# bchess/k8s-1m

Measured on AMD Instinct MI355X. Metric: pods scheduled/sec at 1M nodes (1/2/4/8 GPU) + % of HBM roofline, higher is better.
Workload: dtype int64+f64

## Files before the change

k8s-1m_amd/csrc/ksched_eval.hpp:

```cpp
#pragma once

#include <hip/hip_runtime.h>

#include "ksched_dev.hpp"

namespace ks {

struct NodeRegs {
  double free_cpu, free_mem;
  double rcpu, rmem;
  double lf100_cpu, lf100_mem;
  double acpu_d, amem_d;
  double inv_cpu, inv_mem;
  double bamul;
  uint32_t slot;
  uint32_t bits;
  uint32_t lashift;
};

__device__ __forceinline__ NodeRegs make_regs_inv(int64_t acpu, int64_t amem, int64_t rc, int64_t rm, int64_t zc,
                                                  int64_t zm, int32_t apods, int32_t np, uint32_t slot,
                                                  double inv_cpu, double inv_mem) {
  NodeRegs r;
  r.slot = slot;
// ... 183 lines not shown
  const uint32_t rb = __builtin_amdgcn_readfirstlane(f.rcp_both), rc = __builtin_amdgcn_readfirstlane(f.rcp_cpu),
                 rm = __builtin_amdgcn_readfirstlane(f.rcp_mem);
  const bool hc = r.inv_cpu != 0.0, hm = r.inv_mem != 0.0;
  const uint32_t rcp = hc ? (hm ? rb : rc) : rm;
  return (int32_t)__umulhi(n << 1, rcp);
}

__device__ __forceinline__ uint32_t *fit_table_lds() {
  __shared__ uint32_t s_fit_table[FIT_TABLE_WORDS];
  return s_fit_table;
}
__device__ __forceinline__ void fit_table_stage(const uint32_t *table) {
  if (threadIdx.x < FIT_TABLE_WORDS) fit_table_lds()[threadIdx.x] = table[threadIdx.x];
}
__device__ __forceinline__ int32_t score_fit_rtcr(double nz100_cpu, double nz100_mem, const NodeRegs &r,
                                                  const FitParams &f, const uint8_t *T) {
  const uint32_t uc = min(fit_resource(true, r.lf100_cpu, nz100_cpu, r.acpu_d, r.inv_cpu), 100u);
  const uint32_t um = min(fit_resource(true, r.lf100_mem, nz100_mem, r.amem_d, r.inv_mem), 100u);
  const uint32_t tc = r.inv_cpu != 0.0 ? (uint32_t)T[uc] : 0u, tm = r.inv_mem != 0.0 ? (uint32_t)T[um] : 0u;
  const uint32_t rb = __builtin_amdgcn_readfirstlane(f.rcp_both), rc = __builtin_amdgcn_readfirstlane(f.rcp_cpu),
                 rm = __builtin_amdgcn_readfirstlane(f.rcp_mem);
  return (int32_t)fit_rtcr_node_score(tc, tm, f.wc, f.wm, rc, rm, rb);
}

template <int GF>
__device__ __forceinline__ int32_t score_fit_nz(double nz100_cpu, double nz100_mem, const NodeRegs &r,
                                                const FitParams &f) {
  static_assert(GF == 1 || GF == 2, "the default strategy scores a PodDev (score_la)");
  if constexpr (GF == 2) return score_fit_rtcr(nz100_cpu, nz100_mem, r, f, (const uint8_t *)fit_table_lds());
  else return score_fit_general(nz100_cpu, nz100_mem, r, f);
}
template <int GF>
__device__ __forceinline__ int32_t score_fit(const PodDev &p, const NodeRegs &r, const FitParams &f) {
  if constexpr (GF == 0) return score_la(p, r);
  else return score_fit_nz<GF>(p.nz100_cpu, p.nz100_mem, r, f);
}

template <int GF>
__device__ __forceinline__ void fit_x_resource(FitXSum &x, uint32_t w, int64_t cap, int64_t req, const FitParams &f,
                                               const uint8_t *T) {
  static_assert(GF == 1 || GF == 2, "the default strategy lists no extended resource");
  if constexpr (GF == 2) {
    const uint32_t u = min(fit_x_score(true, cap, req), 100u);
    fit_x_add_rtcr(x, w, cap ? (uint32_t)T[u] : 0u);
  } else {
    fit_x_add(x, w, fit_x_score(f.most != 0, cap, req), cap != 0);
  }
}
template <int GF>
__device__ __forceinline__ int32_t score_fit_x(const PodDev &p, const NodeRegs &r, const FitParams &f, FitXSum x,
                                               const uint32_t *xrcp, const uint8_t *T) {
  if constexpr (GF == 2) {
    const uint32_t uc = min(fit_resource(true, r.lf100_cpu, p.nz100_cpu, r.acpu_d, r.inv_cpu), 100u);
    const uint32_t um = min(fit_resource(true, r.lf100_mem, p.nz100_mem, r.amem_d, r.inv_mem), 100u);
    fit_x_add_rtcr(x, f.wc, r.inv_cpu != 0.0 ? (uint32_t)T[uc] : 0u);
    fit_x_add_rtcr(x, f.wm, r.inv_mem != 0.0 ? (uint32_t)T[um] : 0u);
    return (int32_t)fit_x_round_div(x.n, x.d);
  } else {
    const uint32_t sc = fit_resource(f.most, r.lf100_cpu, p.nz100_cpu, r.acpu_d, r.inv_cpu);
    const uint32_t sm = fit_resource(f.most, r.lf100_mem, p.nz100_mem, r.amem_d, r.inv_mem);
    const uint32_t n = x.n + wmad(f.wc, sc, wmul(f.wm, sm));
    const bool hc = r.inv_cpu != 0.0, hm = r.inv_mem != 0.0;
    const uint32_t rcp = hc ? (hm ? xrcp[3] : xrcp[1]) : (hm ? xrcp[2] : xrcp[0]);
    return (int32_t)fit_x_div(n, rcp);
  }
}

__device__ __forceinline__ double div_rn(double a, double b, double y) {
  const double q0 = a * y;
  const double r = __builtin_fma(-b, q0, a);
  return __builtin_fma(r, y, q0);
}

__device__ __forceinline__ int32_t score_ba_sum(double sc, double sm, const NodeRegs &r) {
  const double f0 = fmin(div_rn(sc, r.acpu_d, r.inv_cpu), 1.0);
  const double f1 = fmin(div_rn(sm, r.amem_d, r.inv_mem), 1.0);
  const double om = __builtin_fma(-fabs(f0 - f1), r.bamul, 1.0);
  return (int32_t)(om * 100.0);
}

__device__ __forceinline__ double ba_fraction(double s, double alloc, double inv) {
  return fmin(div_rn(s, alloc, inv), 1.0);
}
__device__ __forceinline__ int32_t score_ba_fractions(double f0, double f1, const NodeRegs &r) {
  const double om = __builtin_fma(-fabs(f0 - f1), r.bamul, 1.0);
  return (int32_t)(om * 100.0);
}
__device__ __forceinline__ int32_t score_la_cpu(int32_t la_cpu, double nz100_mem, const NodeRegs &r) {
  return (la_cpu + least_requested(r.lf100_mem, nz100_mem, r.inv_mem)) >> r.lashift;
}

__device__ __forceinline__ int32_t score_ba(const PodDev &p, const NodeRegs &r) {
  return score_ba_sum(r.rcpu + p.req_cpu_d, r.rmem + p.req_mem_d, r);
}

__device__ __forceinline__ int64_t taint_raw(const PodDev &p, const NodeExt &e) {
  return (int64_t)__popcll(e.prefer & ~p.tol_prefer);
}

__device__ __forceinline__ int64_t normalize(int64_t raw, int64_t mx, bool reverse) {
  if (mx == 0) return reverse ? 100 : 0;
  const int64_t s = (int64_t)((uint32_t)(100 * raw) / (uint32_t)mx);
  return reverse ? 100 - s : s;
}

template <bool EXT, int GF>
__device__ __forceinline__ int32_t total_score(const PodDev &p, const uint64_t *clauses, const NodeRegs &r,
                                               const NodeExt &e, const Weights &w, const FitParams &fs,
                                               int64_t tt_max, int64_t na_max) {
  int32_t t = (int32_t)wmul((uint32_t)w.fit, (uint32_t)score_fit<GF>(p, r, fs)) +
              (int32_t)wmul((uint32_t)w.ba, (uint32_t)score_ba(p, r));
  int32_t tt = 100;
  if (EXT && (p.flags & PF_TT)) tt = (int32_t)normalize(taint_raw(p, e), tt_max, true);
  t += w.tt * tt;
  if (p.flags & PF_HAS_PREF) {
    int32_t na = 0;
    if (EXT && (p.flags & PF_NA)) na = (int32_t)normalize(preferred_raw(p, clauses, e, r.slot), na_max, false);
    t += (int32_t)wmul((uint32_t)w.na, (uint32_t)na);
  }
  return t;
}

__device__ __forceinline__ uint64_t pack_key(int64_t total, uint32_t slot) {
  return ((uint64_t)(total + 1) << 32) | (uint64_t)(0xFFFFFFFFu - slot);
}

__device__ __forceinline__ void ext_from_words(const uint64_t *w, NodeExt &e) {
  e.hard = w[0];
  e.prefer = w[1];
#pragma unroll
  for (int q = 0; q < LW; ++q) e.lab[q] = w[2 + q];
#pragma unroll
  for (int q = 0; q < NNUM; ++q) e.num[q] = (int64_t)w[2 + LW + q];
}

template <bool EXT>
__device__ __forceinline__ void status_delta(const PodDev &p, const uint64_t *clauses, int st0, int st1,
                                            const NodeExt &e, uint32_t slot, int64_t tt_max, int64_t na_max,
                                            int32_t *d) {
  d[0] += (st0 == ST_FEASIBLE) - (st1 == ST_FEASIBLE);
#pragma unroll
  for (int q = 0; q < NFILT; ++q) d[1 + q] += (st1 == q) - (st0 == q);
  if (EXT && (p.flags & PF_TT)) {
    const int at = taint_raw(p, e) == tt_max;
    d[6] += (st0 == ST_FEASIBLE) * at - (st1 == ST_FEASIBLE) * at;
  }
  if (EXT && (p.flags & PF_NA)) {
    const int at = preferred_raw(p, clauses, e, slot) == na_max;
    d[7] += (st0 == ST_FEASIBLE) * at - (st1 == ST_FEASIBLE) * at;
  }
}

}
```

k8s-1m_amd/csrc/ksched_kernels.hip:

```cpp
#include <hip/hip_runtime.h>

#include <utility>

#include "ksched_dev.hpp"
#include "ksched_eval.hpp"
#include "ksched_kernels.hpp"
#include "ksched_instr.hpp"
#include "ksched_util.hpp"

namespace ks {




typedef unsigned u32x4 __attribute__((ext_vector_type(4)));
typedef const __attribute__((address_space(4))) u32x4 *const_words;
template <bool SCALAR = false>
__device__ __forceinline__ PodDev load_pod(const PodDev *pods, uint32_t i) {
  if constexpr (SCALAR) {
    const const_words src = (const_words)(pods + i);
    u32x4 w[sizeof(PodDev) / 16];
#pragma unroll
    for (int k = 0; k < (int)(sizeof(PodDev) / 16); ++k) w[k] = src[k];
    PodDev p;
    __builtin_memcpy(&p, w, sizeof p);
    return p;
  } else {
    return pods[i];
  }
}


template <typename T>
__device__ __forceinline__ void pin_vgpr(T &x) {
  asm volatile("" : "+v"(x));
}

template <int NPL, int LWU>
__device__ __forceinline__ const uint64_t *term_pass_n(const uint64_t *t, const NodeExt (&e)[NPL],
                                                       const NodeRegs (&nr)[NPL], uint32_t (&ok)[NPL]) {
  const uint64_t w0 = t[0];
  const uint32_t ng = uniform_u32((uint32_t)w0 & 0xFF), nn = uniform_u32(((uint32_t)w0 >> 8) & 0xFF),
                 nm = uniform_u32(((uint32_t)w0 >> 16) & 0xFF);
  uint64_t must[LWU], mf[LWU];
#pragma unroll
  for (int k = 0; k < LWU; ++k) {
    must[k] = t[1 + k];
    mf[k] = t[1 + LW + k];
  }
  static_for<NPL>([&](auto J) {
    constexpr int j = J;
    uint64_t diff = 0;
#pragma unroll
    for (int k = 0; k < LWU; ++k) diff |= (e[j].lab[k] & mf[k]) ^ must[k];
    ok[j] = diff == 0 ? 1u : 0u;
  });
  const uint64_t *g = t + TERM_HDR_WORDS;
  for (uint32_t i = 0; i < ng; ++i, g += LW) {
    uint64_t gm[LWU];
#pragma unroll
    for (int k = 0; k < LWU; ++k) gm[k] = g[k];
    static_for<NPL>([&](auto J) {
      constexpr int j = J;
      uint64_t any = 0;
#pragma unroll
      for (int k = 0; k < LWU; ++k) any |= e[j].lab[k] & gm[k];
      ok[j] &= any != 0 ? 1u : 0u;
    });
  }
  for (uint32_t i = 0; i < nn; ++i, g += 2) {
    const bool col1 = g[0] & 0xFF, gt = ((g[0] >> 8) & 0xFF) == TO_GT;
    const int64_t x = (int64_t)g[1];
    static_for<NPL>([&](auto J) {
      constexpr int j = J;
      const int64_t v = col1 ? e[j].num[1] : e[j].num[0];
      ok[j] &= (gt ? v > x : v < x) ? 1u : 0u;
    });
  }
  for (uint32_t i = 0; i < nm; ++i, g += 2) {
    const bool in = g[0] == TO_NAME_IN;
    const int64_t x = (int64_t)g[1];
    static_for<NPL>([&](auto J) {
      constexpr int j = J;
      ok[j] &= (((int64_t)nr[j].slot == x) == in) ? 1u : 0u;
    });
  }
  return g;
}

template <int NPL, int LWU>
__device__ __forceinline__ void required_match_n(const PodDev &p, const uint64_t *prog, const NodeExt (&e)[NPL],
                                                 const NodeRegs (&nr)[NPL], bool (&out)[NPL]) {
  uint32_t any[NPL];
  static_for<NPL>([&](auto J) { any[J] = 0u; });
  const uint64_t *t = prog + p.req_off;
  for (uint32_t k = 0; k < p.req_len; ++k) {
    uint32_t ok[NPL];
    t = term_pass_n<NPL, LWU>(t, e, nr, ok);
    static_for<NPL>([&](auto J) { any[J] |= ok[J]; });
  }
  static_for<NPL>([&](auto J) { out[J] = any[J] != 0u; });
}

template <int NPL, int LWU>
__device__ __forceinline__ void preferred_raw_n(const PodDev &p, const uint64_t *prog, const NodeExt (&e)[NPL],
                                                const NodeRegs (&nr)[NPL], uint32_t (&raw)[NPL]) {
  static_for<NPL>([&](auto J) { raw[J] = 0u; });
  const uint64_t *t = prog + p.pref_off;
  for (uint32_t k = 0; k < p.pref_len; ++k) {
    const uint32_t w = uniform_u32((uint32_t)(t[0] >> 32));
    uint32_t ok[NPL];
    t = term_pass_n<NPL, LWU>(t, e, nr, ok);
    static_for<NPL>([&](auto J) { raw[J] += ok[J] * w; });
  }
}

constexpr double NORM_EPS = 0x1p-40;
__device__ __forceinline__ uint32_t normalize_inv(uint32_t raw, double inv) {
  return (uint32_t)__builtin_fma((double)(100u * raw), inv, NORM_EPS);
}


constexpr uint32_t KEY32_POS_BITS = 9, KEY32_POS_MASK = (1u << KEY32_POS_BITS) - 1;
static_assert(((uint64_t)KS_MAX_PLUGIN_WEIGHT << KEY32_POS_BITS) < (1ull << 24), "pre-shifted weight: 24-bit operand");
static_assert((((uint64_t)4 * 100 * KS_MAX_PLUGIN_WEIGHT + 1) << KEY32_POS_BITS) + KEY32_POS_MASK < (1ull << 31),
              "the sweep's 32-bit key");

template <int NPL, bool EXT, int LWU = LW, int GF = 0>
__global__ __launch_bounds__(SWEEP_THREADS) __attribute__((amdgpu_waves_per_eu(EXT && NPL == 2 && !GF ? 5 : 1)))
void sweep_kernel(RoundArgs a) {
  static_assert(NPL * WAVE <= (1 << KEY32_POS_BITS), "wave-local key position field");
  constexpr int NW = SWEEP_THREADS / WAVE;
  __shared__ uint64_t s_keys[MAX_PG][NW][3];
  constexpr int NCNT = NFILT + 5;
  __shared__ uint32_t s_cnt[MAX_PG][NW][NCNT];
  __shared__ uint64_t s_stage[EXT ? 1 : NW][EXT ? 1 : WL_T][EXT ? 1 : WL_ROW];

  const uint32_t start = uniform_u32(*a.sstart);
  const uint32_t sh = blockIdx.z;
  const Shard s = a.shards[a.shard0 + sh];
  const uint32_t wid = threadIdx.x / WAVE;
  const uint32_t kw = blockIdx.x * NW + wid;
  const uint32_t kwaves = s.waves * a.sub;
  const uint32_t lane = threadIdx.x % WAVE;
  const uint32_t lwave = kw / a.sub, j0 = (kw % a.sub) * NPL;
  const uint32_t p0 = start + blockIdx.y * a.pg;
  uint32_t p1 = min(min(p0 + a.pg, start + a.P), a.npods);
  const bool fix = EXT && a.fix;
  const bool dedup = !fix && a.ulist != nullptr;
  if (dedup) p1 = min(p1, start + uniform_u32(*a.nuniq));
  if (p0 >= p1 || blockIdx.x * NW >= kwaves) return;
  if (fix && uniform_u32(a.fix_group[blockIdx.y]) == 0) return;
  if constexpr (GF == 2) {
    fit_table_stage(a.fit_table);
    __syncthreads();
  }

  NodeRegs nr[NPL];
  NodeExt ne[EXT ? NPL : 1];
  static_for<NPL>([&](auto J) {
    constexpr int j = J;
    const uint32_t l = (j0 + (uint32_t)j) * WAVE * s.waves + lane * s.waves + lwave;
    const uint32_t pos = s.base + kw * WAVE * NPL + (uint32_t)j * WAVE + lane;
    load_core(a.t, pos, s.lo + l, kw < kwaves && l < s.count, nr[j]);
    if constexpr (EXT) load_ext<LWU>(a.t, pos, nr[j].bits & 1u, ne[j]);
  });

  bool podfit[NPL];
  uint64_t podfit_m[NPL];
  uint32_t vcount = 0;
  static_for<NPL>([&](auto J) {
    constexpr int j = J;
    podfit[j] = nr[j].bits & 2u;
    podfit_m[j] = __builtin_amdgcn_ballot_w64(podfit[j]);
    vcount += popc_ballot(nr[j].bits & 1u);
  });
  const uint32_t kpos0 = KEY32_POS_MASK - lane;
  uint32_t kc[EXT ? 1 : NPL];
  const uint32_t wf9 = (uint32_t)a.w.fit << KEY32_POS_BITS, wb9 = (uint32_t)a.w.ba << KEY32_POS_BITS;
  const uint32_t wt9 = (uint32_t)a.w.tt << KEY32_POS_BITS, wn9 = (uint32_t)a.w.na << KEY32_POS_BITS;
  const uint32_t kpos1 = (1u << KEY32_POS_BITS) + kpos0;
  if constexpr (!EXT) {
    const uint32_t cplus = (uint32_t)(a.w.tt * 100) + 1u;
    static_for<NPL>([&](auto J) { kc[J] = (cplus << KEY32_POS_BITS) + (kpos0 - (uint32_t)J * WAVE); });
  }

  uint32_t feas_v = 0;
  constexpr bool SHARE = !EXT && GF == 0;
  int64_t ck_req = -1, ck_nz = -1;
  double c_f0[SHARE ? NPL : 1];
  int32_t c_la[SHARE ? NPL : 1];
  uint64_t c_fm[SHARE ? NPL : 1];
  static_for<(SHARE ? NPL : 1)>([&](auto J) { c_f0[J] = 0.0; c_la[J] = 0; c_fm[J] = 0; });
  auto sweep_pod = [&](const uint32_t it, const uint32_t q) __attribute__((always_inline)) {
    const uint32_t r = fix ? uniform_u32(a.fix_list[it - start]) : dedup ? uniform_u32(a.ulist[it - start]) : it - start;
    if (fix && r == FIX_NONE) return;
    const uint32_t pi = start + r;
    const PodDev p = load_pod<!EXT>(a.pods, pi);
    uint32_t tt_max = 0, na_max = 0;
    if (EXT && (p.flags & (PF_TT | PF_NA))) {
      tt_max = uniform_u32(fix ? a.norm_max[2 * r + 0] : p.tt_guess);
      na_max = uniform_u32(fix ? a.norm_max[2 * r + 1] : p.na_guess);
    }
    uint32_t b1 = 0, b2 = 0;
    uint32_t feas = 0, f0 = 0, f1 = 0, f2 = 0, f3 = 0, f4 = 0, ttc = 0, nac = 0;
    uint32_t tmx = 0, nmx = 0;
    uint64_t over_m = 0;
    if constexpr (!EXT) {
      const uint64_t zc = __builtin_amdgcn_ballot_w64(p.req_cpu == 0), zm = __builtin_amdgcn_ballot_w64(p.req_mem == 0);
      if constexpr (SHARE) {
        if (p.req_cpu != ck_req || p.nz_cpu != ck_nz) {
          ck_req = p.req_cpu;
          ck_nz = p.nz_cpu;
          static_for<NPL>([&](auto J) {
            constexpr int j = J;
            const double sc = nr[j].rcpu + p.req_cpu_d;
            c_fm[j] = podfit_m[j] & (zc | __builtin_amdgcn_ballot_w64(!(sc > nr[j].acpu_d)));
            c_la[j] = least_requested(nr[j].lf100_cpu, p.nz100_cpu, nr[j].inv_cpu);
            c_f0[j] = ba_fraction(sc, nr[j].acpu_d, nr[j].inv_cpu);
          });
        }
        static_for<NPL>([&](auto J) { pin_vgpr(c_f0[J]); pin_vgpr(c_la[J]); });
        static_for<NPL>([&](auto J) {
          constexpr int j = J;
          const double sm = nr[j].rmem + p.req_mem_d;
          const uint64_t fm = c_fm[j] & (zm | __builtin_amdgcn_ballot_w64(!(sm > nr[j].amem_d)));
          const double f1 = ba_fraction(sm, nr[j].amem_d, nr[j].inv_mem);
          const uint32_t key = sel_mask(fm, wmad_s(wf9, (uint32_t)score_la_cpu(c_la[j], p.nz100_mem, nr[j]),
                                                   wmad_s(wb9, (uint32_t)score_ba_fractions(c_f0[j], f1, nr[j]), kc[j])));
          b2 = max(b2, min(b1, key));
          b1 = max(b1, key);
          feas += (uint32_t)__popcll(fm);
        });
      } else {
        static_for<NPL>([&](auto J) {
          constexpr int j = J;
          const double sc = nr[j].rcpu + p.req_cpu_d, sm = nr[j].rmem + p.req_mem_d;
          const uint64_t fm = podfit_m[j] & (zc | __builtin_amdgcn_ballot_w64(!(sc > nr[j].acpu_d))) &
                              (zm | __builtin_amdgcn_ballot_w64(!(sm > nr[j].amem_d)));
          const uint32_t key = sel_mask(fm, wmad_s(wf9, (uint32_t)score_fit<GF>(p, nr[j], a.fs),
                                                   wmad_s(wb9, (uint32_t)score_ba_sum(sc, sm, nr[j]), kc[j])));
          b2 = max(b2, min(b1, key));
          b1 = max(b1, key);
          feas += (uint32_t)__popcll(fm);
        });
      }
      f4 = vcount - feas;
    } else {
      bool aff[NPL], pre[NPL];
      uint32_t praw[NPL];
      static_for<NPL>([&](auto J) { aff[J] = true; pre[J] = true; praw[J] = 0u; });
      if (p.flags & PF_AFF) required_match_n<NPL, LWU>(p, a.clauses, ne, nr, aff);
      if (p.flags & PF_PREFILTER) {
        static_for<NPL>([&](auto J) { pre[J] = false; });
        for (uint32_t k = 0; k < p.pre_len; ++k) {
          const uint64_t x = a.clauses[p.pre_off + k];
          static_for<NPL>([&](auto J) { pre[J] |= (uint64_t)nr[J].slot == x; });
        }
      }
      const bool conflict = p.flags & PF_NA_CONFLICT;
      if (p.flags & PF_NA) preferred_raw_n<NPL, LWU>(p, a.clauses, ne, nr, praw);
      const double *ip = fix ? a.norm_inv + 2 * r : a.guess_inv + 2 * (size_t)pi;
      const double inv_tt = (p.flags & PF_TT) ? ip[0] : 0.0;
      const double inv_na = (p.flags & PF_NA) ? ip[1] : 0.0;
      const bool hc = p.req_cpu != 0, hm = p.req_mem != 0;
      const bool ext = p.flags & PF_EXT;
      const bool named = p.name_slot != -1;
      static_for<NPL>([&](auto J) {
        constexpr int j = J;
        const bool valid = nr[j].bits & 1u;
        int st = ST_FEASIBLE;
        const double sc = nr[j].rcpu + p.req_cpu_d, sm = nr[j].rmem + p.req_mem_d;
        const bool fitfail = !podfit[j] || (hc && sc > nr[j].acpu_d) || (hm && sm > nr[j].amem_d);
        if (fitfail) st = 4;
        if (ext) {
          const uint64_t untol = ne[j].hard & ~p.tol_hard;
          if (!aff[j]) st = 3;
          if (untol) st = 2;
          if (named && (int64_t)nr[j].slot != (int64_t)p.name_slot) st = 1;
          if (untol & UNSCHED_BIT) st = 0;
          if (conflict) st = 3;
          if (!pre[j]) st = ST_PREFILTERED;
        }
        if (!valid) st = ST_EMPTY;
        const bool feasible = st == ST_FEASIBLE;
        const uint64_t fb = __builtin_amdgcn_ballot_w64(feasible);
        uint32_t acc = kpos1 - (uint32_t)j * WAVE;
        uint32_t tts = 100u;
        if (p.flags & PF_TT) {
          const uint32_t raw = (uint32_t)__popcll(ne[j].prefer & ~p.tol_prefer);
          tts = 100u - normalize_inv(raw, inv_tt);
          ttc += (uint32_t)__popcll(__builtin_amdgcn_ballot_w64(raw == tt_max) & fb);
          over_m |= __builtin_amdgcn_ballot_w64(raw > tt_max) & fb;
          tmx = max(tmx, feasible ? raw : 0u);
        }
        acc = wmad_s(wt9, tts, acc);
        if (p.flags & PF_NA) {
          const uint32_t nas = normalize_inv(praw[j], inv_na);
          nac += (uint32_t)__popcll(__builtin_amdgcn_ballot_w64(praw[j] == na_max) & fb);
          over_m |= __builtin_amdgcn_ballot_w64(praw[j] > na_max) & fb;
          nmx = max(nmx, feasible ? praw[j] : 0u);
          acc = wmad_s(wn9, nas, acc);
        }
        acc = wmad_s(wb9, (uint32_t)score_ba_sum(sc, sm, nr[j]), acc);
        acc = wmad_s(wf9, (uint32_t)score_fit<GF>(p, nr[j], a.fs), acc);
        const uint32_t key = sel_mask(fb, acc);
        b2 = max(b2, min(b1, key));
        b1 = max(b1, key);
        const uint64_t vb = __builtin_amdgcn_ballot_w64(valid);
        feas += (uint32_t)__popcll(fb);
        if (fb != vb) {
          f0 += popc_ballot(st == 0);
          f1 += popc_ballot(st == 1);
          f2 += popc_ballot(st == 2);
          f3 += popc_ballot(st == 3);
          f4 += popc_ballot(st == 4);
        }
      });
    }
    if (EXT && (p.flags & (PF_TT | PF_NA))) {
      const bool exceeded = over_m != 0;
      if (p.flags & PF_TT) tmx = (!exceeded && ttc) ? tt_max : wave_max_u32_dpp(tmx);
      if (p.flags & PF_NA) nmx = (!exceeded && nac) ? na_max : wave_max_u32_dpp(nmx);
    }
    if constexpr (!EXT) {
      s_stage[wid][q][lane] = (uint64_t)b2 << 32 | b1;
      feas_v = writelane_u32(feas_v, feas, q);
      return;
    }
    const uint32_t best = b1, second = b2;
    uint32_t bound32 = wave_max_u32_dpp(second);
    uint32_t c = best > bound32 ? best : 0u;
    const uint32_t ncand = popc_ballot(c != 0u);
    uint32_t c1 = 0, c2 = 0;
    if (ncand) {
      c1 = wave_max_u32_dpp(c);
      if (ncand > 1) {
        if (c == c1) c = 0;
        c2 = wave_max_u32_dpp(c);
        if (ncand > 2) {
          if (c == c2) c = 0;
          bound32 = max(bound32, wave_max_u32_dpp(c));
        }
      }
    }
    if (lane == 0) {
      auto widen = [&](uint32_t k) -> uint64_t {
        if (!k) return 0ull;
        const uint32_t q = KEY32_POS_MASK - (k & KEY32_POS_MASK);
        const uint32_t slot = s.lo + (j0 + q / WAVE) * WAVE * s.waves + (q % WAVE) * s.waves + lwave;
        return ((uint64_t)(k >> KEY32_POS_BITS) << 32) | (uint64_t)(0xFFFFFFFFu - slot);
      };
      const uint64_t k1 = widen(c1), k2 = widen(c2), bound = widen(bound32);
      const uint32_t pl = it - p0;
      s_keys[pl][wid][0] = k1;
      s_keys[pl][wid][1] = k2;
      s_keys[pl][wid][2] = bound;
      s_cnt[pl][wid][0] = feas;
      s_cnt[pl][wid][1] = f0;
      s_cnt[pl][wid][2] = f1;
      s_cnt[pl][wid][3] = f2;
      s_cnt[pl][wid][4] = f3;
      s_cnt[pl][wid][5] = f4;
      s_cnt[pl][wid][6] = ttc;
      s_cnt[pl][wid][7] = nac;
      s_cnt[pl][wid][8] = tmx;
      s_cnt[pl][wid][9] = nmx;
    }
  };
  if constexpr (EXT) {
    for (uint32_t it = p0; it < p1; ++it) sweep_pod(it, 0u);
  } else {
    const uint32_t bq = lane % WL_T, bg = lane / WL_T;
    for (uint32_t b0 = p0; b0 < p1; b0 += WL_T) {
      const uint32_t nb = min((uint32_t)WL_T, p1 - b0);
#pragma nounroll
      for (uint32_t q = 0; q < nb; ++q) sweep_pod(b0 + q, q);
      wave_lds_order();
      WaveTuple w = {0u, 0u, 0u, 0u};
      static_for<WL_SEG>([&](auto I) {
        const uint64_t v = s_stage[wid][bq][bg * WL_SEG + (uint32_t)I];
        wl_fold(w, (uint32_t)v, (uint32_t)(v >> 32));
      });
      wave_lds_order();
      w = wl_merge(w, tuple_ror8(w));
      w = wl_merge(w, tuple_xor(w, 16));
      w = wl_merge(w, tuple_xor(w, 32));
      const uint32_t pl = b0 - p0 + bq;
      if (bq < nb) {
        if (bg < 3) {
          const uint32_t k = wl_entry(w, bg);
          const uint32_t kq = KEY32_POS_MASK - (k & KEY32_POS_MASK);
          const uint32_t slot = s.lo + (j0 + kq / WAVE) * WAVE * s.waves + (kq % WAVE) * s.waves + lwave;
          s_keys[pl][wid][bg] = k ? ((uint64_t)(k >> KEY32_POS_BITS) << 32) | (uint64_t)(0xFFFFFFFFu - slot) : 0ull;
        }
        static_assert(NCNT == 10 && WL_T == 8, "counter words over the segments");
        s_cnt[pl][wid][bg < 5 ? bg : bg + 1] = bg == 0 ? feas_v : 0u;
        if (bg == 0) {
          s_cnt[pl][wid][5] = vcount - feas_v;
          s_cnt[pl][wid][9] = 0u;
        }
      }
    }
  }
  __syncthreads();
  const uint32_t npl = p1 - p0;
  for (uint32_t pl = threadIdx.x; pl < npl; pl += blockDim.x) {
    const uint32_t r = fix ? a.fix_list[p0 + pl - start] : dedup ? a.ulist[p0 + pl - start] : p0 + pl - start;
    if (fix && r == FIX_NONE) continue;
    uint64_t k[2 * NW];
    uint64_t bound = 0;
    const uint32_t nwaves = min((uint32_t)NW, kwaves - blockIdx.x * NW);
    static_for<NW>([&](auto W) {
      constexpr int w = W;
      const bool on = (uint32_t)w < nwaves;
      k[2 * w] = on ? s_keys[pl][w][0] : 0ull;
      k[2 * w + 1] = on ? s_keys[pl][w][1] : 0ull;
      const uint64_t b = on ? s_keys[pl][w][2] : 0ull;
      bound = b > bound ? b : bound;
    });
    sort8_desc(k);
    bound = max(bound, k[BLOCK_KEYS]);
    const uint32_t nk = 2 * NW;
    BlockRec br;
#pragma unroll
    for (int i = 0; i < BLOCK_KEYS; ++i) br.keys[i] = (i < (int)nk && k[i] > bound) ? k[i] : 0ull;
    br.bound = bound;
    uint32_t cnt[NFILT + 3] = {0, 0, 0, 0, 0, 0, 0, 0};
    uint32_t tmx = 0, nmx = 0;
    for (uint32_t w = 0; w < nwaves; ++w) {
      for (int q = 0; q < NFILT + 3; ++q) cnt[q] += s_cnt[pl][w][q];
      tmx = max(tmx, s_cnt[pl][w][8]);
      nmx = max(nmx, s_cnt[pl][w][9]);
    }
    br.feasible = cnt[0];
    for (int q = 0; q < NFILT; ++q) br.fails[q] = cnt[1 + q];
    br.tt_cnt = cnt[6];
    br.na_cnt = cnt[7];
    br.tt_max = tmx;
    br.na_max = nmx;
    if (EXT && a.pstat_sweep && !fix && cnt[0]) {
      uint32_t *pm = &a.pstat[r].tt_max;
      const uint64_t cur = __hip_atomic_load((uint64_t *)pm, __ATOMIC_RELAXED, __HIP_MEMORY_SCOPE_AGENT);
      if (tmx + 1u > (uint32_t)cur) atomicMax(pm, tmx + 1u);
      if (nmx + 1u > (uint32_t)(cur >> 32)) atomicMax(pm + 1, nmx + 1u);
    }
    a.brec[((size_t)sh * a.P + r) * a.bstride + blockIdx.x] = br;
  }
}

__device__ void bitonic_desc(uint64_t *s, uint32_t m) {
  for (uint32_t k = 2; k <= m; k <<= 1) {
    for (uint32_t j = k >> 1; j > 0; j >>= 1) {
      for (uint32_t p = threadIdx.x; p < m / 2; p += blockDim.x) {
        const uint32_t i = ((p & ~(j - 1)) << 1) | (p & (j - 1));
        const uint64_t x = s[i], y = s[i + j];
        const bool desc = (i & k) == 0;
        if (desc ? (x < y) : (x > y)) { s[i] = y; s[i + j] = x; }
      }
      __syncthreads();
// ... 206 lines not shown
    h->na_cnt = nac;
    for (int z = 0; z < NFILT; ++z) h->fails[z] = fl[z];
  }
}

__device__ __forceinline__ CandRow cand_row(int64_t acpu, int64_t amem, int64_t rc, int64_t rm, int64_t zc, int64_t zm,
                                            int32_t apods, int32_t np, uint32_t pos) {
  CandRow w;
  w.acpu = (double)acpu;
  w.amem = (double)amem;
  w.inv_cpu = acpu ? 1.0 / w.acpu : 0.0;
  w.inv_mem = amem ? 1.0 / w.amem : 0.0;
  w.rc = (double)rc;
  w.rm = (double)rm;
  w.zc100 = (double)zc * 100.0;
  w.zm100 = (double)zm * 100.0;
  w.apods = apods;
  w.np = np;
  w.pos = pos;
  w._pad = 0;
  return w;
}

template <bool EXT>
__global__ __launch_bounds__(256) void gather_cand_kernel(RoundArgs a) {
  const uint32_t start = uniform_u32(*a.sstart);
  const uint32_t r = blockIdx.x;
  if (start + r >= a.npods || r >= a.P) return;
  if (a.rep != nullptr && a.rep[r] != r) return;
  const uint64_t *rec = a.frec + (size_t)r * rec_words(a.K);
  const uint32_t nk = ((const ShardRecHdr *)rec)->nkeys;
  for (uint32_t t = threadIdx.x; t < nk; t += blockDim.x) {
    const uint64_t k = rec[REC_HDR_WORDS + t];
    const uint32_t pos = a.slot_pos[0xFFFFFFFFu - (uint32_t)k];
    a.crow[(size_t)r * a.K + t] = cand_row(a.t.acpu[pos], a.t.amem[pos], a.t.rcpu[pos], a.t.rmem[pos], a.t.zcpu[pos],
                                           a.t.zmem[pos], a.t.apods[pos], a.t.npods[pos], pos);
    if (EXT) {
      CandExt x;
      x.w[0] = a.t.hard[pos];
      x.w[1] = a.t.prefer[pos];
#pragma unroll
      for (int q = 0; q < LW; ++q) x.w[2 + q] = a.t.lab[(size_t)q * a.t.npos + pos];
#pragma unroll
      for (int q = 0; q < NNUM; ++q) x.w[2 + LW + q] = (uint64_t)a.t.num[(size_t)q * a.t.npos + pos];
      a.cext[(size_t)r * a.K + t] = x;
    }
  }
}

constexpr int PHASH = 1024;
static_assert(2 * MAX_P >= MAX_K, "patch thread counts");


__device__ __forceinline__ uint32_t count_greater(const uint64_t *v, uint32_t n, uint64_t x) {
  uint32_t lo = 0, hi = n;
  while (lo < hi) {
    const uint32_t mid = (lo + hi) >> 1;
    if (v[mid] > x) lo = mid + 1;
    else hi = mid;
  }
  return lo;
}


template <bool EXT, int PATCH_THREADS, int GF = 0>
__global__ __launch_bounds__(PATCH_THREADS) void patch_kernel(RoundArgs a) {
  static_assert(PATCH_THREADS >= MAX_P, "one thread per carried node");
  constexpr int NW = PATCH_THREADS / WAVE;
  __shared__ uint32_t s_hkey[PHASH];
  __shared__ uint64_t s_k1[MAX_P];
  __shared__ uint64_t s_ckey[MAX_P];
  __shared__ uint64_t s_lkey[MAX_K];
  __shared__ uint32_t s_wl[NW], s_wc[NW];
  __shared__ int32_t s_wd[NW][NFILT + 3];
  __shared__ uint64_t s_wdrop[NW];

  const uint32_t tid = threadIdx.x, lane = tid % WAVE, wid = tid / WAVE;
  const uint32_t start = uniform_u32(*a.act);
  const uint32_t r = blockIdx.x;
  if (a.first || start >= a.npods || uniform_u32(*a.sstart) != start || start + r >= a.npods) return;
  if (a.rep != nullptr && uniform_u32(a.rep[r]) != r) return;
  const uint32_t nc = uniform_u32(*a.carry_in_n);
  if (nc == 0) return;
  const PodDev p = load_pod(a.pods, start + r);
  uint64_t *rec = a.frec + (size_t)r * rec_words(a.K);
  ShardRecHdr *hdr = (ShardRecHdr *)rec;
  const uint64_t bound = hdr->bound;
  const uint32_t nk = hdr->nkeys;
  int64_t tt_max = 0, na_max = 0;
  if (EXT) {
    tt_max = a.norm_max[2 * r];
    na_max = a.norm_max[2 * r + 1];
  }
  for (uint32_t i = tid; i < PHASH; i += PATCH_THREADS) s_hkey[i] = 0;
  if constexpr (GF == 2) fit_table_stage(a.fit_table);
  __syncthreads();

  int32_t d[NFILT + 3] = {0, 0, 0, 0, 0, 0, 0, 0};
  uint64_t k1 = 0;
  if (tid < nc) {
    const CarryRec &cr = a.carry_in[tid];
    NodeExt ce{};
    if (EXT) ext_from_words(cr.ext, ce);
    const double inv_cpu = cr.acpu ? 1.0 / (double)cr.acpu : 0.0, inv_mem = cr.amem ? 1.0 / (double)cr.amem : 0.0;
    const NodeRegs r1 = make_regs_inv(cr.acpu, cr.amem, cr.rc, cr.rm, cr.zc, cr.zm, cr.apods, cr.np, cr.slot,
                                      inv_cpu, inv_mem);
    NodeRegs r0 = r1;
    r0.free_cpu = (double)(cr.acpu - cr.rc0);
    r0.free_mem = (double)(cr.amem - cr.rm0);
    r0.bits = (r1.bits & ~2u) | ((int64_t)cr.np0 + 1 <= (int64_t)cr.apods ? 2u : 0u);
    const int st0 = filter<EXT>(p, a.clauses, r0, ce);
    const int st1 = filter<EXT>(p, a.clauses, r1, ce);
    if (st1 == ST_FEASIBLE) k1 = pack_key(total_score<EXT, GF>(p, a.clauses, r1, ce, a.w, a.fs, tt_max, na_max), cr.slot);
    if (st0 != st1) status_delta<EXT>(p, a.clauses, st0, st1, ce, cr.slot, tt_max, na_max, d);
    uint32_t h = rhash(cr.slot);
    while (atomicCAS(&s_hkey[h], 0u, cr.slot + 1) != 0u) h = (h + 1) & (PHASH - 1);
  }
  if (tid < MAX_P) s_k1[tid] = k1;
  if (__ballot(d[0] | d[1] | d[2] | d[3] | d[4] | d[5] | d[6] | d[7]) != 0) {
#pragma unroll
    for (int q = 0; q < NFILT + 3; ++q) d[q] = wave_sum_i32_dpp(d[q]);
  }
  if (lane == 0)
    for (int q = 0; q < NFILT + 3; ++q) s_wd[wid][q] = d[q];
  __syncthreads();

  static_assert(sizeof(CandRow) == 80 && sizeof(CandExt) == 64, "patch row pieces");
  uint64_t lk = 0;
  bool keep = false;
  uint4 lr0, lr1, lr2, lr3, lr4, lx0, lx1, lx2, lx3;
  if (tid < nk) {
    lk = rec[REC_HDR_WORDS + tid];
    const uint32_t slot = 0xFFFFFFFFu - (uint32_t)lk;
    uint32_t h = rhash(slot);
    keep = true;
    while (s_hkey[h] != 0) {
      if (s_hkey[h] == slot + 1) { keep = false; break; }
      h = (h + 1) & (PHASH - 1);
    }
    if (keep) {
      const uint4 *sr = (const uint4 *)&a.crow[(size_t)r * a.K + tid];
      lr0 = sr[0], lr1 = sr[1], lr2 = sr[2], lr3 = sr[3], lr4 = sr[4];
      if (EXT) {
        const uint4 *sx = (const uint4 *)&a.cext[(size_t)r * a.K + tid];
        lx0 = sx[0], lx1 = sx[1], lx2 = sx[2], lx3 = sx[3];
      }
    }
  }
  const bool cin = k1 > bound;
  const uint64_t kb = __ballot(keep), cb = __ballot(cin);
  const uint64_t lt = (1ull << lane) - 1ull;
  if (lane == 0) {
    s_wl[wid] = (uint32_t)__popcll(kb);
    s_wc[wid] = (uint32_t)__popcll(cb);
  }
  __syncthreads();
  uint32_t li = (uint32_t)__popcll(kb & lt), nsurv = 0, ncl = 0;
#pragma unroll
  for (int w = 0; w < NW; ++w) {
    li += (uint32_t)w < wid ? s_wl[w] : 0u;
    nsurv += s_wl[w];
    ncl += s_wc[w];
  }
  uint32_t crank = 0;
  if (cin) {
    for (uint32_t c = 0; c < nc; ++c) crank += s_k1[c] > k1;
    s_ckey[crank] = k1;
// ... 473 lines not shown
```

k8s-1m_amd/csrc/ksched_util.hpp:

```cpp
#pragma once

#include <hip/hip_runtime.h>

#include <utility>

#include "ksched_dev.hpp"
#include "ksched_eval.hpp"

namespace ks {

constexpr int KS_PLUGIN_FIT_IDX = 4;
typedef __attribute__((address_space(1))) void gvoid_t;
typedef __attribute__((address_space(3))) void lvoid_t;

template <class F, int... I>
__device__ __forceinline__ void static_for_impl(F &&f, std::integer_sequence<int, I...>) {
  (f(std::integral_constant<int, I>{}), ...);
}
template <int N, class F>
__device__ __forceinline__ void static_for(F &&f) {
  static_for_impl(f, std::make_integer_sequence<int, N>{});
}

__device__ __forceinline__ uint64_t wave_max_u64(uint64_t v) {
#pragma unroll
  for (int m = 32; m >= 1; m >>= 1) {
    uint64_t o = __shfl_xor(v, m, WAVE);
    v = o > v ? o : v;
  }
  return v;
}

__device__ __forceinline__ void cx_desc(uint64_t &a, uint64_t &b) {
  const uint64_t hi = a > b ? a : b, lo = a > b ? b : a;
  a = hi;
  b = lo;
}
__device__ __forceinline__ void sort8_desc(uint64_t *k) {
  cx_desc(k[0], k[2]); cx_desc(k[1], k[3]); cx_desc(k[4], k[6]); cx_desc(k[5], k[7]);
  cx_desc(k[0], k[4]); cx_desc(k[1], k[5]); cx_desc(k[2], k[6]); cx_desc(k[3], k[7]);
  cx_desc(k[0], k[1]); cx_desc(k[2], k[3]); cx_desc(k[4], k[5]); cx_desc(k[6], k[7]);
  cx_desc(k[2], k[4]); cx_desc(k[3], k[5]);
  cx_desc(k[1], k[4]); cx_desc(k[3], k[6]);
  cx_desc(k[1], k[2]); cx_desc(k[3], k[4]); cx_desc(k[5], k[6]);
}

__device__ __forceinline__ uint32_t popc_ballot(bool b) {
  return (uint32_t)__popcll(__builtin_amdgcn_ballot_w64(b));
}

__device__ __forceinline__ uint32_t sel_mask(uint64_t m, uint32_t v) {
  uint32_t r;
  asm("v_cndmask_b32_e64 %0, 0, %1, %2" : "=v"(r) : "v"(v), "s"(m));
  return r;
}

__device__ __forceinline__ uint32_t uniform_u32(uint32_t v) {
  return __builtin_amdgcn_readfirstlane(v);
}

__device__ __forceinline__ uint32_t smax_u32(uint32_t a, uint32_t b) {
  uint32_t r;
  asm("s_max_u32 %0, %1, %2" : "=s"(r) : "s"(a), "s"(b) : "scc");
  return r;
}

template <int CTRL>
__device__ __forceinline__ uint32_t dpp32(uint32_t v) {
  return (uint32_t)__builtin_amdgcn_update_dpp(0, (int)v, CTRL, 0xF, 0xF, false);
}
template <int CTRL>
__device__ __forceinline__ uint64_t dpp64(uint64_t v) {
  return ((uint64_t)dpp32<CTRL>((uint32_t)(v >> 32)) << 32) | dpp32<CTRL>((uint32_t)v);
}
__device__ __forceinline__ uint64_t max64(uint64_t a, uint64_t b) { return a > b ? a : b; }
__device__ __forceinline__ uint64_t readlane64(uint64_t v, int l) {
  return ((uint64_t)(uint32_t)__builtin_amdgcn_readlane((int)(v >> 32), l) << 32) |
         (uint32_t)__builtin_amdgcn_readlane((int)(uint32_t)v, l);
}
__device__ __forceinline__ uint64_t max8_u64(uint64_t v) {
  v = max64(v, dpp64<0xB1>(v));
  v = max64(v, dpp64<0x4E>(v));
  return max64(v, dpp64<0x141>(v));
}
__device__ __forceinline__ uint64_t wave_max_u64_dpp(uint64_t v) {
  v = max8_u64(v);
  v = max64(v, dpp64<0x140>(v));
  return max64(max64(readlane64(v, 0), readlane64(v, 16)), max64(readlane64(v, 32), readlane64(v, 48)));
}
__device__ __forceinline__ uint32_t wave_max_u32_dpp(uint32_t v) {
  v = max(v, dpp32<0xB1>(v));
  v = max(v, dpp32<0x4E>(v));
  v = max(v, dpp32<0x141>(v));
  v = max(v, dpp32<0x140>(v));
  return smax_u32(smax_u32((uint32_t)__builtin_amdgcn_readlane((int)v, 0), (uint32_t)__builtin_amdgcn_readlane((int)v, 16)),
                  smax_u32((uint32_t)__builtin_amdgcn_readlane((int)v, 32), (uint32_t)__builtin_amdgcn_readlane((int)v, 48)));
}
__device__ __forceinline__ uint32_t writelane_u32(uint32_t v, uint32_t x, uint32_t l) {
#pragma clang diagnostic push
#pragma clang diagnostic ignored "-Winline-asm"
  asm("s_mov_b32 m0, %2\n\tv_writelane_b32 %0, %1, m0" : "+v"(v) : "s"(x), "s"(l) : "m0");
#pragma clang diagnostic pop
  return v;
}
__device__ __forceinline__ void wave_lds_order() {
  __builtin_amdgcn_fence(__ATOMIC_RELEASE, "wavefront");
  __builtin_amdgcn_wave_barrier();
  __builtin_amdgcn_fence(__ATOMIC_ACQUIRE, "wavefront");
}
__device__ __forceinline__ WaveTuple tuple_ror8(const WaveTuple &w) {
  return {dpp32<0x128>(w.t1), dpp32<0x128>(w.t2), dpp32<0x128>(w.t3), dpp32<0x128>(w.B)};
}
__device__ __forceinline__ WaveTuple tuple_xor(const WaveTuple &w, int m) {
  return {(uint32_t)__shfl_xor((int)w.t1, m, WAVE), (uint32_t)__shfl_xor((int)w.t2, m, WAVE),
          (uint32_t)__shfl_xor((int)w.t3, m, WAVE), (uint32_t)__shfl_xor((int)w.B, m, WAVE)};
}
__device__ __forceinline__ uint32_t min8_u32(uint32_t v) {
  v = min(v, dpp32<0xB1>(v));
  v = min(v, dpp32<0x4E>(v));
  return min(v, dpp32<0x141>(v));
}
__device__ __forceinline__ int32_t sum8_i32(int32_t v) {
  v += (int32_t)dpp32<0xB1>((uint32_t)v);
  v += (int32_t)dpp32<0x4E>((uint32_t)v);
  return v + (int32_t)dpp32<0x141>((uint32_t)v);
}
__device__ __forceinline__ int32_t wave_sum_i32_dpp(int32_t v) {
  v = sum8_i32(v);
  v += (int32_t)dpp32<0x140>((uint32_t)v);
  return __builtin_amdgcn_readlane(v, 0) + __builtin_amdgcn_readlane(v, 16) + __builtin_amdgcn_readlane(v, 32) +
         __builtin_amdgcn_readlane(v, 48);
}

__device__ __forceinline__ void stall_for(uint32_t usec) {
  const uint64_t t0 = __builtin_amdgcn_s_memrealtime();
  while (__builtin_amdgcn_s_memrealtime() - t0 < 100ull * usec) __builtin_amdgcn_s_sleep(127);
}

__device__ __forceinline__ void signal_done(uint32_t *flag, uint32_t seq, uint32_t stall_us = 0) {
  if (flag == nullptr) return;
  if (stall_us) stall_for(stall_us);
  __threadfence_system();
  __hip_atomic_store(flag, seq, __ATOMIC_RELEASE, __HIP_MEMORY_SCOPE_SYSTEM);
}

__device__ __forceinline__ void mark_pod(uint8_t *marks, uint32_t i, uint8_t bit) {
// ... 82 lines not shown
```

Measured before the change: 886,200.

## Prefetch next pod's request fields via scalar loads in non-EXT sweep

The non-EXT sweep now loads only the f64 request fields of each pod through scalar constant loads and software-pipelines them, double-buffering the next pod's load while the current one is scored. The dedup list is read once per lane and broadcast with readlane. Zero-request masks become scalar compares, and the clamp to 1.0 in the balanced-allocation fraction is applied only when the request is zero. Per-kernel waves-per-EU hints are also retuned. The intent is to hide per-pod load latency and cut VALU work. The risks are hand-written waitcnt encoding and the assumption that the PodDev field layout stays fixed.

Result: faster. 971,400, median of 6 (+9.6%).

```diff
diff --git a/k8s-1m_amd/csrc/ksched_eval.hpp b/k8s-1m_amd/csrc/ksched_eval.hpp
--- a/k8s-1m_amd/csrc/ksched_eval.hpp
+++ b/k8s-1m_amd/csrc/ksched_eval.hpp
@@ -289,6 +289,8 @@
 __device__ __forceinline__ double ba_fraction(double s, double alloc, double inv) {
   return fmin(div_rn(s, alloc, inv), 1.0);
 }
+__device__ __forceinline__ double ba_quotient(double s, double alloc, double inv) { return div_rn(s, alloc, inv); }
+__device__ __forceinline__ double ba_clamp(double q) { return fmin(q, 1.0); }
 __device__ __forceinline__ int32_t score_ba_fractions(double f0, double f1, const NodeRegs &r) {
   const double om = __builtin_fma(-fabs(f0 - f1), r.bamul, 1.0);
   return (int32_t)(om * 100.0);
diff --git a/k8s-1m_amd/csrc/ksched_kernels.hip b/k8s-1m_amd/csrc/ksched_kernels.hip
--- a/k8s-1m_amd/csrc/ksched_kernels.hip
+++ b/k8s-1m_amd/csrc/ksched_kernels.hip
@@ -15,20 +15,17 @@
 
 typedef unsigned u32x4 __attribute__((ext_vector_type(4)));
 typedef const __attribute__((address_space(4))) u32x4 *const_words;
-template <bool SCALAR = false>
-__device__ __forceinline__ PodDev load_pod(const PodDev *pods, uint32_t i) {
-  if constexpr (SCALAR) {
-    const const_words src = (const_words)(pods + i);
-    u32x4 w[sizeof(PodDev) / 16];
-#pragma unroll
-    for (int k = 0; k < (int)(sizeof(PodDev) / 16); ++k) w[k] = src[k];
-    PodDev p;
-    __builtin_memcpy(&p, w, sizeof p);
-    return p;
-  } else {
-    return pods[i];
-  }
-}
+__device__ __forceinline__ PodDev load_pod_requests(const PodDev *pods, uint32_t i) {
+  static_assert(offsetof(PodDev, req_cpu_d) == 32 && offsetof(PodDev, nz100_cpu) == 48 &&
+                offsetof(PodDev, tol_hard) == 64, "PodDev: the binary64 request fields");
+  const const_words src = (const_words)(pods + i);
+  const u32x4 w2 = src[2], w3 = src[3];
+  PodDev p = {};
+  __builtin_memcpy(&p.req_cpu_d, &w2, 16);
+  __builtin_memcpy(&p.nz100_cpu, &w3, 16);
+  return p;
+}
+__device__ __forceinline__ uint64_t f64_bits(double x) { return (uint64_t)__double_as_longlong(x); }
 
 
 template <typename T>
@@ -127,7 +124,7 @@
               "the sweep's 32-bit key");
 
 template <int NPL, bool EXT, int LWU = LW, int GF = 0>
-__global__ __launch_bounds__(SWEEP_THREADS) __attribute__((amdgpu_waves_per_eu(EXT && NPL == 2 && !GF ? 5 : 1)))
+__global__ __launch_bounds__(SWEEP_THREADS) __attribute__((amdgpu_waves_per_eu(EXT ? (NPL == 2 && !GF ? 5 : 1) : NPL == 8 ? 2 : NPL == 4 && !GF ? 4 : 1)))
 void sweep_kernel(RoundArgs a) {
   static_assert(NPL * WAVE <= (1 << KEY32_POS_BITS), "wave-local key position field");
   constexpr int NW = SWEEP_THREADS / WAVE;
@@ -187,16 +184,12 @@
 
   uint32_t feas_v = 0;
   constexpr bool SHARE = !EXT && GF == 0;
-  int64_t ck_req = -1, ck_nz = -1;
+  uint64_t ck_req = ~0ull, ck_nz = ~0ull;
   double c_f0[SHARE ? NPL : 1];
   int32_t c_la[SHARE ? NPL : 1];
   uint64_t c_fm[SHARE ? NPL : 1];
   static_for<(SHARE ? NPL : 1)>([&](auto J) { c_f0[J] = 0.0; c_la[J] = 0; c_fm[J] = 0; });
-  auto sweep_pod = [&](const uint32_t it, const uint32_t q) __attribute__((always_inline)) {
-    const uint32_t r = fix ? uniform_u32(a.fix_list[it - start]) : dedup ? uniform_u32(a.ulist[it - start]) : it - start;
-    if (fix && r == FIX_NONE) return;
-    const uint32_t pi = start + r;
-    const PodDev p = load_pod<!EXT>(a.pods, pi);
+  auto sweep_pod = [&](const uint32_t it, const uint32_t q, const uint32_t r, const PodDev &p) __attribute__((always_inline)) {
     uint32_t tt_max = 0, na_max = 0;
     if (EXT && (p.flags & (PF_TT | PF_NA))) {
       tt_max = uniform_u32(fix ? a.norm_max[2 * r + 0] : p.tt_guess);
@@ -207,30 +200,51 @@
     uint32_t tmx = 0, nmx = 0;
     uint64_t over_m = 0;
     if constexpr (!EXT) {
-      const uint64_t zc = __builtin_amdgcn_ballot_w64(p.req_cpu == 0), zm = __builtin_amdgcn_ballot_w64(p.req_mem == 0);
+      uint64_t zc, zm;
+      const uint64_t rq_cpu = f64_bits(p.req_cpu_d), rq_mem = f64_bits(p.req_mem_d), nz_cpu = f64_bits(p.nz100_cpu);
       if constexpr (SHARE) {
-        if (p.req_cpu != ck_req || p.nz_cpu != ck_nz) {
-          ck_req = p.req_cpu;
-          ck_nz = p.nz_cpu;
+        zc = uniform_zero_mask(rq_cpu);
+        zm = uniform_zero_mask(rq_mem);
+      } else {
+        zc = __builtin_amdgcn_ballot_w64(rq_cpu == 0);
+        zm = __builtin_amdgcn_ballot_w64(rq_mem == 0);
+      }
+      if constexpr (SHARE) {
+        if (rq_cpu != ck_req || nz_cpu != ck_nz) {
+          ck_req = rq_cpu;
+          ck_nz = nz_cpu;
           static_for<NPL>([&](auto J) {
             constexpr int j = J;
             const double sc = nr[j].rcpu + p.req_cpu_d;
             c_fm[j] = podfit_m[j] & (zc | __builtin_amdgcn_ballot_w64(!(sc > nr[j].acpu_d)));
             c_la[j] = least_requested(nr[j].lf100_cpu, p.nz100_cpu, nr[j].inv_cpu);
-            c_f0[j] = ba_fraction(sc, nr[j].acpu_d, nr[j].inv_cpu);
+            c_f0[j] = ba_quotient(sc, nr[j].acpu_d, nr[j].inv_cpu);
           });
+          if (rq_cpu == 0) {
+            static_for<NPL>([&](auto J) { c_f0[J] = ba_clamp(c_f0[J]); });
+            asm volatile("");
+          }
         }
         static_for<NPL>([&](auto J) { pin_vgpr(c_f0[J]); pin_vgpr(c_la[J]); });
+        double f1[NPL];
+        uint64_t fm[NPL];
         static_for<NPL>([&](auto J) {
           constexpr int j = J;
           const double sm = nr[j].rmem + p.req_mem_d;
-          const uint64_t fm = c_fm[j] & (zm | __builtin_amdgcn_ballot_w64(!(sm > nr[j].amem_d)));
-          const double f1 = ba_fraction(sm, nr[j].amem_d, nr[j].inv_mem);
-          const uint32_t key = sel_mask(fm, wmad_s(wf9, (uint32_t)score_la_cpu(c_la[j], p.nz100_mem, nr[j]),
-                                                   wmad_s(wb9, (uint32_t)score_ba_fractions(c_f0[j], f1, nr[j]), kc[j])));
+          fm[j] = c_fm[j] & (zm | __builtin_amdgcn_ballot_w64(!(sm > nr[j].amem_d)));
+          f1[j] = ba_quotient(sm, nr[j].amem_d, nr[j].inv_mem);
+        });
+        if (rq_mem == 0) {
+          static_for<NPL>([&](auto J) { f1[J] = ba_clamp(f1[J]); });
+          asm volatile("");
+        }
+        static_for<NPL>([&](auto J) {
+          constexpr int j = J;
+          const uint32_t key = sel_mask(fm[j], wmad_s(wf9, (uint32_t)score_la_cpu(c_la[j], p.nz100_mem, nr[j]),
+                                                      wmad_s(wb9, (uint32_t)score_ba_fractions(c_f0[j], f1[j], nr[j]), kc[j])));
           b2 = max(b2, min(b1, key));
           b1 = max(b1, key);
-          feas += (uint32_t)__popcll(fm);
+          feas += (uint32_t)__popcll(fm[j]);
         });
       } else {
         static_for<NPL>([&](auto J) {
@@ -260,7 +274,7 @@
       }
       const bool conflict = p.flags & PF_NA_CONFLICT;
       if (p.flags & PF_NA) preferred_raw_n<NPL, LWU>(p, a.clauses, ne, nr, praw);
-      const double *ip = fix ? a.norm_inv + 2 * r : a.guess_inv + 2 * (size_t)pi;
+      const double *ip = fix ? a.norm_inv + 2 * r : a.guess_inv + 2 * (size_t)(start + r);
       const double inv_tt = (p.flags & PF_TT) ? ip[0] : 0.0;
       const double inv_na = (p.flags & PF_NA) ? ip[1] : 0.0;
       const bool hc = p.req_cpu != 0, hm = p.req_mem != 0;
@@ -369,13 +383,51 @@
     }
   };
   if constexpr (EXT) {
-    for (uint32_t it = p0; it < p1; ++it) sweep_pod(it, 0u);
+    for (uint32_t it = p0; it < p1; ++it) {
+      const uint32_t r = fix ? uniform_u32(a.fix_list[it - start]) : dedup ? uniform_u32(a.ulist[it - start]) : it - start;
+      if (fix && r == FIX_NONE) continue;
+      const PodDev p = a.pods[start + r];
+      sweep_pod(it, 0u, r, p);
+    }
   } else {
+    static_assert(MAX_PG <= WAVE && WL_T % 2 == 0, "one list entry per lane; batches start on pa");
     const uint32_t bq = lane % WL_T, bg = lane / WL_T;
+    uint32_t ev = p0 - start + lane;
+    if (dedup && lane < p1 - p0) ev = a.ulist[ev];
+    auto load_ahead = [&](const uint32_t it, PodDev &p) __attribute__((always_inline)) {
+      if (it < p1) p = load_pod_requests(a.pods, start + (uint32_t)__builtin_amdgcn_readlane((int)ev, (int)(it - p0)));
+    };
+    auto in_use = [&](const PodDev &p) __attribute__((always_inline)) { asm volatile("" ::"s"(f64_bits(p.req_cpu_d))); };
+    auto arrived = [&](const PodDev &p) __attribute__((always_inline)) {
+      __builtin_amdgcn_s_waitcnt(0xC07F);
+      in_use(p);
+    };
+    PodDev pa = {}, pb = {};
+    load_ahead(p0, pa);
     for (uint32_t b0 = p0; b0 < p1; b0 += WL_T) {
-      const uint32_t nb = min((uint32_t)WL_T, p1 - b0);
+      const uint32_t nb = smin_u32((uint32_t)WL_T, p1 - b0);
+      if constexpr (GF == 0) {
 #pragma nounroll
-      for (uint32_t q = 0; q < nb; ++q) sweep_pod(b0 + q, q);
+        for (uint32_t q = 0;;) {
+          in_use(pa);
+          load_ahead(b0 + q + 1, pb);
+          sweep_pod(b0 + q, q, 0u, pa);
+          arrived(pb);
+          if (++q >= nb) break;
+          load_ahead(b0 + q + 1, pa);
+          sweep_pod(b0 + q, q, 0u, pb);
+          arrived(pa);
+          if (++q >= nb) break;
+        }
+      } else {
+#pragma nounroll
+        for (uint32_t q = 0; q < nb; ++q) {
+          pb = pa;
+          load_ahead(b0 + q + 1, pa);
+          sweep_pod(b0 + q, q, 0u, pb);
+          arrived(pa);
+        }
+      }
       wave_lds_order();
       WaveTuple w = {0u, 0u, 0u, 0u};
       static_for<WL_SEG>([&](auto I) {
@@ -748,7 +800,7 @@
   if (a.rep != nullptr && uniform_u32(a.rep[r]) != r) return;
   const uint32_t nc = uniform_u32(*a.carry_in_n);
   if (nc == 0) return;
-  const PodDev p = load_pod(a.pods, start + r);
+  const PodDev p = a.pods[start + r];
   uint64_t *rec = a.frec + (size_t)r * rec_words(a.K);
   ShardRecHdr *hdr = (ShardRecHdr *)rec;
   const uint64_t bound = hdr->bound;
diff --git a/k8s-1m_amd/csrc/ksched_util.hpp b/k8s-1m_amd/csrc/ksched_util.hpp
--- a/k8s-1m_amd/csrc/ksched_util.hpp
+++ b/k8s-1m_amd/csrc/ksched_util.hpp
@@ -62,6 +62,17 @@
 __device__ __forceinline__ uint32_t smax_u32(uint32_t a, uint32_t b) {
   uint32_t r;
   asm("s_max_u32 %0, %1, %2" : "=s"(r) : "s"(a), "s"(b) : "scc");
+  return r;
+}
+
+__device__ __forceinline__ uint32_t smin_u32(uint32_t a, uint32_t b) {
+  uint32_t r;
+  asm("s_min_u32 %0, %1, %2" : "=s"(r) : "s"(a), "s"(b) : "scc");
+  return r;
+}
+__device__ __forceinline__ uint64_t uniform_zero_mask(uint64_t x) {
+  uint64_t r;
+  asm("s_cmp_eq_u64 %1, 0\n\ts_cselect_b64 %0, -1, 0" : "=s"(r) : "s"(x) : "scc");
   return r;
 }
 
```
